# klausondrag/FOSVOS

Measured on AMD Instinct MI355X. Metric: online fine-tune frames/sec (854x480), higher is better.
Workload: dtype bf16; 1 GPU; OSVOS_VGG train_online one-shot fine-tune: 1x3x480x854 frame per step, fwd + class-balanced BCE + bwd, fused SGD step every 5 steps (BASELINE.json configs[1]); batch=1, avg_grad_every_n=5, activations=bf16 NHWC, fp32 accumulate, fp32 master weights, parallelism=single GPU

## Files before the change

### fosvos_amd/csrc/common.hpp

```cpp
#pragma once
#include <hip/hip_runtime.h>
#include <stdarg.h>
#include <algorithm>
#include <stdint.h>
#include <stdio.h>
#include <stdlib.h>
#include <string.h>

#include "../../include/fosvos_hip.h"

namespace fosvos {

extern thread_local char g_err[512];

inline int fail(int code, const char *fmt, ...) __attribute__((format(printf, 2, 3)));
inline int fail(int code, const char *fmt, ...) {
    va_list ap;
    va_start(ap, fmt);
    vsnprintf(g_err, sizeof(g_err), fmt, ap);
    va_end(ap);
    return code;
}

#define FOSVOS_HIP_CHECK(expr)                                                                         \
    do {                                                                                               \
        hipError_t e_ = (expr);                                                                        \
        if (e_ != hipSuccess)                                                                          \
            return ::fosvos::fail(FOSVOS_E_HIP, "%s: %s (%s:%d)", #expr, hipGetErrorString(e_), __FILE__, \
                                  __LINE__);                                                           \
    } while (0)

#define FOSVOS_REQUIRE(cond, code, ...)                    \
    do {                                                   \
        if (!(cond)) return ::fosvos::fail(code, __VA_ARGS__); \
    } while (0)

#define FOSVOS_ENTER(device) FOSVOS_HIP_CHECK(hipSetDevice(device))
extern bool g_prof_on;
void prof_begin(const char *name, hipStream_t st, double flops);
void prof_end();
#define FOSVOS_PROF(name, st, flops)                                        \
    do {                                                                    \
        if (::fosvos::g_prof_on) ::fosvos::prof_begin(name, (hipStream_t)(st), flops); \
    } while (0)
#define FOSVOS_LAUNCH_CHECK()                            \
    do {                                                 \
        if (::fosvos::g_prof_on) ::fosvos::prof_end();   \
        FOSVOS_HIP_CHECK(hipGetLastError());             \
    } while (0)

struct WgradReduceEntry {
    const float *slabs;
    float *dw, *db;
    const float *bias_part;
    int64_t E_real, E_pad;
    int S, S_bias, Co, Cor, accumulate;
    int block_begin, n_blocks;
    int fold_begin, fold_blocks;
};
constexpr int kWgradReduceMax = 20;
struct WgradReduceTable {
    int n;
    WgradReduceEntry e[kWgradReduceMax];
};
int wgrad_impl(const uint16_t *x, const uint16_t *dy, float *dw, float *db, int N, int H, int W, int Ci, int Co,
               int accumulate, void *workspace, size_t workspace_bytes, int device, void *stream,
               WgradReduceTable *reduce, bool alone = false);
int first_wgrad_impl(const float *frame, const uint16_t *dy, float *dw, float *db, int N, int H, int W, int Co,
                     int accumulate, void *workspace, size_t workspace_bytes, int device, void *stream,
                     WgradReduceTable *reduce);
int wgrad_reduce_all(WgradReduceTable *reduce, int device, void *stream);
int wgrad_queue_reduce(const float *slabs, const float *bias_part, float *dw, float *db, int S, int S_bias, int64_t E_real,
                       int64_t E_pad, int Co, int Cor, int accumulate, WgradReduceTable *reduce, int device, void *stream);
struct HeadBwdArgs {
    const float *const *side;
    const int *hs, *ws;
    const float *const *filt, *const *filt1;
    const float *dsn_w, *fuse_w, *d_fused;
    const float *const *d_side_out;
    uint16_t *const *d_side;
    float *d_fuse_w, *d_fuse_b, *d_dsn_w, *d_dsn_b;
    int N, H, W, accumulate;
    void *workspace;
    size_t workspace_bytes;
    int device;
    int filt_uniform;
};
int head_bwd_check(const HeadBwdArgs &a);
int head_bwd_scale(const HeadBwdArgs &a, int s, void *stream);
int head_bwd_finish(const HeadBwdArgs &a, void *stream);

}
constexpr int kFosvosVggEvents = 25, kFosvosResnetEvents = 12;
struct fosvos_ctx {
    uint32_t magic;
    int device;
    hipEvent_t vgg_ev[kFosvosVggEvents];
    hipEvent_t resnet_ev[kFosvosResnetEvents];
    bool buckets_recorded;
};
constexpr uint32_t kFosvosCtxMagic = 0x58544346u;
namespace fosvos {
inline int ctx_check(const fosvos_ctx *ctx, const char *who) {
    FOSVOS_REQUIRE(ctx != nullptr, FOSVOS_E_ARG, "%s: null context (fosvos_ctx_create)", who);
    FOSVOS_REQUIRE(ctx->magic == kFosvosCtxMagic, FOSVOS_E_ARG, "%s: not a live fosvos_ctx", who);
    return FOSVOS_OK;
}

#ifdef FOSVOS_LAB_BUILD
inline const char *lab_env(const char *name) { return getenv(name); }
#else
// ... 158 lines not shown
```

### fosvos_amd/csrc/conv_wgrad.hip

```cpp
#include <stdlib.h>

#include "common.hpp"

using namespace fosvos;

namespace {
constexpr int TH = 8;
constexpr int TPIX = TH * 16;
constexpr int HALO_W = 18;
constexpr int BCI = 64;

struct WgArgs {
    const uint16_t *x;
    const uint16_t *dy;
    float *slabs;
    float *bias_part;
    int N, H, W, Ci, Cy, Cor;
    int tiles_x, tiles_y, n_tiles, tiles_per_split;
    int lab;
    int S, n_ci, n_co, xcd_order;
};

typedef __attribute__((address_space(3))) s16x4 *lds_s16x4_ptr;

// ... 205 lines not shown
            if constexpr ((R) < 4) {                                                                                \
                _Pragma("unroll") for (int kx = 0; kx < 3; ++kx)                                                    \
                _Pragma("unroll") for (int u = 0; u < NU; ++u)                                                      \
                    acc[kx][u] = __builtin_amdgcn_mfma_f32_16x16x32_bf16(a0[u], b[kx], acc[kx][u], 0, 0, 0);        \
                if (my_bias) {                                                                                      \
                    _Pragma("unroll") for (int u = 0; u < NU; ++u) bsum[u] = add8(a0[u], bsum[u]);                  \
                }                                                                                                   \
            }                                                                                                       \
            asm volatile("" ::: "memory");                                                                          \
            b[0] = bn[0]; b[1] = bn[1]; b[2] = bn[2];                                                               \
        }
        FOSVOS_W2_ROW(0) FOSVOS_W2_ROW(1) FOSVOS_W2_ROW(2) FOSVOS_W2_ROW(3) FOSVOS_W2_ROW(4) FOSVOS_W2_ROW(5)
        if (has_next) FOSVOS_W2_ADVANCE()
        asm volatile("s_waitcnt vmcnt(0)" ::: "memory");
        __syncthreads();
    }

    if (do_bias) {
        float *sb = reinterpret_cast<float *>(smem_w);
#pragma unroll
        for (int u = 0; u < NU; ++u) sb[(wi * 4 + g) * C::BCO + wc * 32 + u * 16 + (lane & 15)] = bsum[u];
        __syncthreads();
        if (tid < C::BCO && co0 + tid < a.Cor) {
            float acc_b = 0.f;
#pragma unroll
            for (int k = 0; k < 16; ++k) acc_b += sb[k * C::BCO + tid];
            a.bias_part[((int64_t)split * a.n_ci + ci_blk) * a.Cor + co0 + tid] = acc_b;
        }
    }
    float *slab = a.slabs + (int64_t)split * a.Cor * a.Ci * 9;
    const int ci = ci0 + wi * 16 + (lane & 15);
#pragma unroll
    for (int u = 0; u < NU; ++u)
#pragma unroll
        for (int r = 0; r < 4; ++r) {
            const int co = co0 + wc * 32 + u * 16 + 4 * g + r;
            if (co >= a.Cor || (a.lab & 1)) continue;
            float *d = slab + ((int64_t)co * a.Ci + ci) * 9;
#pragma unroll
            for (int t = 0; t < 9; ++t) d[t] = acc[t][u][r];
        }
#undef FOSVOS_W2_ROW
#undef FOSVOS_W2_PIECES_OF_ROW
#undef FOSVOS_W2_PIECE_ANY
#undef FOSVOS_W2_TILE_SCALARS
#undef FOSVOS_W2_ADVANCE
#undef FOSVOS_W2_STAGE
#undef FOSVOS_W2_PIECE_X
#undef FOSVOS_W2_PIECE_Y
}
}

constexpr int kFold = 8;

__global__ __launch_bounds__(256) void k_wgrad_fold(const WgradReduceTable t) {
    int e = 0;
    while (e + 1 < t.n && (int)blockIdx.x >= t.e[e + 1].fold_begin) ++e;
    const WgradReduceEntry &q = t.e[e];
    const int local = blockIdx.x - q.fold_begin;
    if (local >= q.fold_blocks) return;
    const int per_group = q.n_blocks;
    const int grp = local / per_group;
    const int64_t i4 = (int64_t)(local - grp * per_group) * 256 + threadIdx.x;
    if (i4 * 4 >= q.E_real) return;
    float *base = const_cast<float *>(q.slabs) + (int64_t)grp * kFold * q.E_pad + i4 * 4;
    const int n = min(kFold, q.S - grp * kFold);
    float4 v[kFold];
#pragma unroll
    for (int j = 0; j < kFold; ++j) v[j] = *reinterpret_cast<const float4 *>(base + (int64_t)min(j, n - 1) * q.E_pad);
    float4 acc = v[0];
#pragma unroll
    for (int j = 1; j < kFold; ++j)
        if (j < n) { acc.x += v[j].x; acc.y += v[j].y; acc.z += v[j].z; acc.w += v[j].w; }
    *reinterpret_cast<float4 *>(base) = acc;
}

__global__ __launch_bounds__(256) void k_wgrad_reduce(const WgradReduceTable t) {
    int e = 0;
    while (e + 1 < t.n && (int)blockIdx.x >= t.e[e + 1].block_begin) ++e;
    const WgradReduceEntry &q = t.e[e];
    const int local = blockIdx.x - q.block_begin;
    const int64_t i4 = (int64_t)local * 256 + threadIdx.x;
    const bool folded = q.fold_blocks > 0;
    const int n_src = folded ? (q.S + kFold - 1) / kFold : q.S;
    const int64_t stride = (folded ? kFold : 1) * q.E_pad;
    if (i4 * 4 < q.E_real) {
        const float *src = q.slabs + i4 * 4;
        float4 acc = make_float4(0.f, 0.f, 0.f, 0.f);
        for (int s0 = 0; s0 < n_src; s0 += 8) {
            float4 v[8];
#pragma unroll
            for (int j = 0; j < 8; ++j) v[j] = *reinterpret_cast<const float4 *>(src + (int64_t)min(s0 + j, n_src - 1) * stride);
#pragma unroll
            for (int j = 0; j < 8; ++j)
                if (s0 + j < n_src) { acc.x += v[j].x; acc.y += v[j].y; acc.z += v[j].z; acc.w += v[j].w; }
        }
        float4 *d = reinterpret_cast<float4 *>(q.dw + i4 * 4);
        if (q.accumulate) {
            const float4 o = *d;
            acc.x += o.x; acc.y += o.y; acc.z += o.z; acc.w += o.w;
        }
        *d = acc;
    }
    if (local == 0 && q.db) {
        __shared__ float s_part[256];
        int Cg = 1;
        while (Cg < q.Co && Cg < 256) Cg <<= 1;
        const int P = 256 / Cg, part = threadIdx.x / Cg, cl = threadIdx.x - part * Cg;
        const int per = (q.S_bias + P - 1) / P, s_lo = part * per, s_hi = min(s_lo + per, q.S_bias);
        for (int co0 = 0; co0 < q.Co; co0 += Cg) {
            const int co = co0 + cl;
            float acc_b = 0.f;
            if (co < q.Co) {
                for (int s0 = s_lo; s0 < s_hi; s0 += 16) {
                    float v[16];
#pragma unroll
                    for (int j = 0; j < 16; ++j) v[j] = q.bias_part[(int64_t)min(s0 + j, s_hi - 1) * q.Cor + co];
#pragma unroll
                    for (int j = 0; j < 16; ++j)
                        if (s0 + j < s_hi) acc_b += v[j];
                }
            }
            if (co0) __syncthreads();
            s_part[threadIdx.x] = acc_b;
            __syncthreads();
            if (part == 0 && co < q.Co) {
                float t = s_part[cl];
                for (int pp = 1; pp < P; ++pp) t += s_part[pp * Cg + cl];
                q.db[co] = q.accumulate ? q.db[co] + t : t;
            }
        }
    }
}

int target_blocks() {
    static const int v = [] {
        const char *e = lab_env("FOSVOS_WGRAD_BLOCKS");
        const int n = e ? atoi(e) : 0;
        return n > 0 ? n : 192;
    }();
    return v;
}

struct Plan {
    int Cor, Cy, side, tiles_x, tiles_y, n_tiles, tps, S, n_ci;
    size_t slab_bytes, bias_bytes;
};

Plan make_plan(int N, int H, int W, int Ci, int Co, bool alone = false) {
    Plan p;
    p.side = Co % 64 != 0;
    p.Cor = p.side ? Co : roundup(Co, 64);
    p.Cy = roundup(Co, 32);
    p.tiles_x = (int)cdiv(W, 16);
    p.tiles_y = (int)cdiv(H, TH);
    p.n_tiles = p.tiles_x * p.tiles_y * N;
    const int out_blocks = p.side ? Ci / 64 : (p.Cor / 64) * (Ci / 64);
    int S = (int)cdiv(alone ? std::max(256, target_blocks()) : target_blocks(), out_blocks);
    if (S > p.n_tiles) S = p.n_tiles;
    if (S < 1) S = 1;
    p.tps = (int)cdiv(p.n_tiles, S);
    p.S = (int)cdiv(p.n_tiles, p.tps);
    p.slab_bytes = (size_t)p.S * 9 * p.Cor * Ci * sizeof(float);
    p.n_ci = Ci / 64;
    p.bias_bytes = (size_t)p.S * p.n_ci * p.Cor * sizeof(float);
    return p;
}

int check_shape(int N, int H, int W, int Ci, int Co, const char *who) {
    FOSVOS_REQUIRE(N > 0 && H > 0 && W > 0 && Ci > 0 && Co > 0, FOSVOS_E_SHAPE, "%s: bad shape", who);
    FOSVOS_REQUIRE(Ci % BCI == 0, FOSVOS_E_SHAPE, "%s: Ci=%d must be a multiple of %d", who, Ci, BCI);
    FOSVOS_REQUIRE(Co % 64 == 0 || Co == 16, FOSVOS_E_SHAPE, "%s: Co=%d must be a multiple of 64, or 16 (side_prep)", who, Co);
    FOSVOS_REQUIRE(((int64_t)N * H * W + W + 1) * std::max(Ci, roundup(Co, 32)) * 2 < 0xffffffffLL, FOSVOS_E_SHAPE,
                   "%s: a tensor of %d x %d x %d x %d bf16 exceeds the 4 GB a buffer descriptor addresses", who, N, H, W,
                   std::max(Ci, roundup(Co, 32)));
    return FOSVOS_OK;
}

int finish_or_queue(const Plan &p, float *slabs, float *bias_part, float *dw, float *db, int Ci, int Co, int accumulate,
                    WgradReduceTable *reduce, int device, hipStream_t st) {
    return fosvos::wgrad_queue_reduce(slabs, bias_part, dw, db, p.S, p.S * p.n_ci, 9LL * Co * Ci, 9LL * p.Cor * Ci, Co, p.Cor,
                                      accumulate, reduce, device, st);
}
}

extern "C" size_t fosvos_conv3x3_wgrad_workspace_bytes(int N, int H, int W, int Ci, int Co) {
    if (N <= 0 || H <= 0 || W <= 0 || Ci <= 0 || Co <= 0 || Ci % BCI != 0) return 0;
    const Plan p = make_plan(N, H, W, Ci, Co), q = make_plan(N, H, W, Ci, Co, true);
    return std::max(p.slab_bytes + p.bias_bytes, q.slab_bytes + q.bias_bytes);
}

extern "C" int fosvos_conv3x3_wgrad(const uint16_t *x, const uint16_t *dy, float *dw, float *db, int N, int H, int W,
                                    int Ci, int Co, int accumulate, void *workspace, size_t workspace_bytes, int device,
                                    void *stream) {
    return fosvos::wgrad_impl(x, dy, dw, db, N, H, W, Ci, Co, accumulate, workspace, workspace_bytes, device, stream,
                              nullptr);
}

extern "C" int fosvos_conv3x3_wgrad_reduce(float *dw, float *db, int N, int H, int W, int Ci, int Co, int accumulate,
                                           void *workspace, size_t workspace_bytes, int device, void *stream) {
    FOSVOS_REQUIRE(dw && workspace, FOSVOS_E_ARG, "conv3x3_wgrad_reduce: null pointer");
    if (int rc = check_shape(N, H, W, Ci, Co, "conv3x3_wgrad_reduce")) return rc;
    const Plan p = make_plan(N, H, W, Ci, Co);
    FOSVOS_REQUIRE(workspace_bytes >= p.slab_bytes + p.bias_bytes, FOSVOS_E_WORKSPACE,
                   "conv3x3_wgrad_reduce: workspace %zu < %zu", workspace_bytes, p.slab_bytes + p.bias_bytes);
    FOSVOS_ENTER(device);
    float *slabs = reinterpret_cast<float *>(workspace);
    float *bias_part = reinterpret_cast<float *>(reinterpret_cast<char *>(workspace) + p.slab_bytes);
    return finish_or_queue(p, slabs, bias_part, dw, db, Ci, Co, accumulate, nullptr, device, (hipStream_t)stream);
}

extern "C" int fosvos_conv3x3_wgrad_slabs(const uint16_t *x, const uint16_t *dy, int with_bias, int N, int H, int W, int Ci,
                                          int Co, void *workspace, size_t workspace_bytes, int device, void *stream) {
    WgradReduceTable sink;
    sink.n = 0;
    float dummy = 0.f;
    return fosvos::wgrad_impl(x, dy, &dummy, with_bias ? &dummy : nullptr, N, H, W, Ci, Co, 0, workspace, workspace_bytes,
                              device, stream, &sink);
}

int fosvos::wgrad_queue_reduce(const float *slabs, const float *bias_part, float *dw, float *db, int S, int S_bias,
                               int64_t E_real,
                               int64_t E_pad, int Co, int Cor, int accumulate, WgradReduceTable *reduce, int device,
                               void *stream) {
    WgradReduceTable local;
    local.n = 0;
    WgradReduceTable *t = reduce ? reduce : &local;
    FOSVOS_REQUIRE(t->n < kWgradReduceMax, FOSVOS_E_ARG, "wgrad: reduction queue full");
    FOSVOS_REQUIRE(E_real % 4 == 0 && E_pad % 4 == 0, FOSVOS_E_SHAPE, "wgrad: slab size must be a multiple of 4 floats");
    WgradReduceEntry &q = t->e[t->n];
    q.slabs = slabs; q.dw = dw; q.db = db; q.bias_part = db ? bias_part : nullptr;
    q.S = S; q.S_bias = S_bias; q.Co = Co; q.Cor = Cor; q.accumulate = accumulate;
    q.E_real = E_real;
    q.E_pad = E_pad;
    q.n_blocks = (int)cdiv(E_real / 4, 256);
    q.block_begin = t->n ? t->e[t->n - 1].block_begin + t->e[t->n - 1].n_blocks : 0;
    q.fold_blocks = S > kFold ? (int)cdiv(S, kFold) * q.n_blocks : 0;
    q.fold_begin = t->n ? t->e[t->n - 1].fold_begin + t->e[t->n - 1].fold_blocks : 0;
    ++t->n;
    return reduce ? FOSVOS_OK : fosvos::wgrad_reduce_all(t, device, stream);
}

int fosvos::wgrad_reduce_all(WgradReduceTable *reduce, int device, void *stream) {
    FOSVOS_REQUIRE(reduce, FOSVOS_E_ARG, "wgrad_reduce_all: null table");
    if (reduce->n == 0) return FOSVOS_OK;
    FOSVOS_ENTER(device);
    const WgradReduceEntry &last = reduce->e[reduce->n - 1];
    if (last.fold_begin + last.fold_blocks > 0) {
        FOSVOS_PROF("k_wgrad_fold", stream, 0.0);
        hipLaunchKernelGGL(k_wgrad_fold, dim3((unsigned)(last.fold_begin + last.fold_blocks)), dim3(256), 0,
                           (hipStream_t)stream, *reduce);
        FOSVOS_LAUNCH_CHECK();
    }
    FOSVOS_PROF("k_wgrad_reduce", stream, 0.0);
    hipLaunchKernelGGL(k_wgrad_reduce, dim3((unsigned)(last.block_begin + last.n_blocks)), dim3(256), 0, (hipStream_t)stream,
                       *reduce);
    FOSVOS_LAUNCH_CHECK();
    reduce->n = 0;
    return FOSVOS_OK;
}

int fosvos::wgrad_impl(const uint16_t *x, const uint16_t *dy, float *dw, float *db, int N, int H, int W, int Ci, int Co,
                       int accumulate, void *workspace, size_t workspace_bytes, int device, void *stream,
                       WgradReduceTable *reduce, bool alone) {
    FOSVOS_REQUIRE(x && dy && dw && workspace, FOSVOS_E_ARG, "conv3x3_wgrad: null pointer");
    if (int rc = check_shape(N, H, W, Ci, Co, "conv3x3_wgrad")) return rc;
    const Plan p = make_plan(N, H, W, Ci, Co, alone);
    FOSVOS_REQUIRE(workspace_bytes >= p.slab_bytes + p.bias_bytes, FOSVOS_E_WORKSPACE,
                   "conv3x3_wgrad: workspace %zu < %zu", workspace_bytes, p.slab_bytes + p.bias_bytes);
    FOSVOS_ENTER(device);
    hipStream_t st = (hipStream_t)stream;
    WgArgs a;
    a.x = x; a.dy = dy; a.slabs = reinterpret_cast<float *>(workspace);
    a.bias_part = db ? reinterpret_cast<float *>(reinterpret_cast<char *>(workspace) + p.slab_bytes) : nullptr;
    a.N = N; a.H = H; a.W = W; a.Ci = Ci; a.Cy = p.Cy; a.Cor = p.Cor;
    a.tiles_x = p.tiles_x; a.tiles_y = p.tiles_y; a.n_tiles = p.n_tiles; a.tiles_per_split = p.tps;
    a.S = p.S; a.n_ci = Ci / 64; a.n_co = p.side ? 1 : p.Cor / 64;
    {
#ifdef FOSVOS_LAB_BUILD
        static const int lab = lab_env_int("FOSVOS_WGRAD_LAB", 0);
        a.lab = lab;
#else
        a.lab = 0;
#endif
        const char *e = lab_env("FOSVOS_WGRAD_XCD");
        a.xcd_order = !(e && atoi(e) == 0);
    }
    static bool once[64][2];
    const double flops = 2.0 * N * H * W * 9.0 * Ci * Co;
    const dim3 grid((unsigned)(p.S * a.n_ci * a.n_co));
    if (p.side) {
        using C2 = v2::Cfg2<true>;
        if (device >= 0 && device < 64 && !once[device][1]) {
            FOSVOS_HIP_CHECK(hipFuncSetAttribute(reinterpret_cast<const void *>(v2::k_wgrad3x3_v2<true>),
                                                 hipFuncAttributeMaxDynamicSharedMemorySize, C2::LDS_BYTES));
            once[device][1] = true;
        }
        FOSVOS_PROF("k_wgrad3x3_v2<true>", st, flops);
        hipLaunchKernelGGL(v2::k_wgrad3x3_v2<true>, grid, dim3(C2::NT), C2::LDS_BYTES, st, a);
    } else {
        using C2 = v2::Cfg2<false>;
        if (device >= 0 && device < 64 && !once[device][0]) {
            FOSVOS_HIP_CHECK(hipFuncSetAttribute(reinterpret_cast<const void *>(v2::k_wgrad3x3_v2<false>),
                                                 hipFuncAttributeMaxDynamicSharedMemorySize, C2::LDS_BYTES));
            once[device][0] = true;
        }
        FOSVOS_PROF("k_wgrad3x3_v2<false>", st, flops);
        hipLaunchKernelGGL(v2::k_wgrad3x3_v2<false>, grid, dim3(C2::NT), C2::LDS_BYTES, st, a);
    }
// ... 4 lines not shown
```

### fosvos_amd/fosvos_hip/__init__.py

```python
from __future__ import annotations

import ctypes
import os
import threading
from ctypes import POINTER, c_char_p, c_float, c_int, c_int64, c_size_t, c_uint, c_void_p

_HERE = os.path.dirname(os.path.abspath(__file__))
PKG_ROOT = os.path.dirname(_HERE)
LIB_PATH = os.environ.get("FOSVOS_HIP_LIB") or os.path.join(PKG_ROOT, "lib", "libfosvos_hip.so")
HEADER_PATH = os.path.join(os.path.dirname(PKG_ROOT), "include", "fosvos_hip.h")

ABI_VERSION = 33
CONV_RELU = 1
CONV_OUT_F32 = 2
VGG_COMPACT_STAGE1 = 1


class FosvosHipError(RuntimeError):
    pass


class SgdEntry(ctypes.Structure):
    _fields_ = [("param", c_void_p), ("grad", c_void_p), ("momentum_buf", c_void_p), ("numel", c_int64),
                ("lr", c_float), ("weight_decay", c_float)]
# ... 54 lines not shown
                ("kind", c_int)]


class ResnetBlock(ctypes.Structure):
    _fields_ = [("conv", Conv2dDesc * 3), ("n_convs", c_int), ("has_down", c_int), ("down", Conv2dDesc)]


class ResnetNet(ctypes.Structure):
    _fields_ = [("first_w", c_void_p), ("first_b", c_void_p), ("first_co", c_int), ("first_fp32_math", c_int), ("first_unfused", c_int),
                ("blocks_per_stage", c_int * 4),
                ("blocks", POINTER(ResnetBlock)), ("side", Conv2dDesc * 4), ("filt", c_void_p * 4),
                ("filt1", c_void_p * 4), ("stride", c_int * 4), ("dsn_w", c_void_p), ("dsn_b", c_void_p),
                ("fuse_b", c_void_p)]

SIGNATURES = {
    "fosvos_abi_version": (c_int, []),
    "fosvos_last_error": (c_char_p, []),
    "fosvos_build_arch": (c_char_p, []),
    "fosvos_ctx_create": (c_int, [c_int, POINTER(c_void_p)]),
    "fosvos_ctx_destroy": (c_int, [c_void_p]),
    "fosvos_ctx_device": (c_int, [c_void_p]),
    "fosvos_conv3x3_plan": (c_int, [c_int, c_int, c_int, c_int, c_int, POINTER(Conv3x3PlanInfo)]),
    "fosvos_conv3x3_fwd_plan": (c_int, [c_int, c_int, c_int, c_int, c_int, ctypes.c_uint, POINTER(Conv3x3PlanInfo)]),
    "fosvos_conv3x3_first_plan": (c_int, [c_int, c_int, c_int, POINTER(c_int), POINTER(c_int)]),
    "fosvos_nchw_f32_to_nhwc_bf16": (c_int, [c_void_p, c_void_p, c_int, c_int, c_int, c_int, c_int, c_int, c_void_p]),
    "fosvos_nhwc_bf16_to_nchw_f32": (c_int, [c_void_p, c_void_p, c_int, c_int, c_int, c_int, c_int, c_int, c_void_p]),
    "fosvos_nhwc_f32_to_nchw_f32": (c_int, [c_void_p, c_void_p, c_int, c_int, c_int, c_int, c_int, c_void_p]),
    "fosvos_nchw_f32_to_nhwc_f32": (c_int, [c_void_p, c_void_p, c_int, c_int, c_int, c_int, c_int, c_void_p]),
    "fosvos_pack_conv3x3_weights": (c_int, [c_void_p, c_int, c_int, c_void_p, c_void_p, c_int, c_void_p]),
    "fosvos_packed_weight_elems": (c_size_t, [c_int, c_int]),
    "fosvos_pack_conv3x3_weights_multi": (c_int, [POINTER(PackEntry), c_int, c_int, c_void_p]),
    "fosvos_conv3x3_first_fwd": (c_int, [c_void_p, c_void_p, c_void_p, c_void_p, c_void_p, c_int, c_int, c_int, c_int, c_int,
                                         c_void_p]),
    "fosvos_conv3x3_dgrad_bits": (c_int, [c_void_p, c_void_p, c_void_p, c_void_p, c_void_p, c_int, c_int, c_int, c_int,
                                          c_int, c_void_p, c_size_t, c_int, c_void_p]),
    "fosvos_conv3x3_dgrad_unpool": (c_int, [c_void_p, c_void_p, c_void_p, c_void_p, c_void_p, c_int, c_int, c_int, c_int,
                                            c_int, c_void_p, c_size_t, c_int, c_void_p]),
    "fosvos_conv3x3_first_wgrad": (c_int, [c_void_p, c_void_p, c_void_p, c_void_p, c_int, c_int, c_int, c_int,
                                           c_void_p, c_size_t, c_int, c_void_p]),
    "fosvos_conv3x3_first_wgrad_workspace_bytes": (c_size_t, [c_int, c_int, c_int, c_int]),
    "fosvos_conv3x3_fwd": (c_int, [c_void_p, c_void_p, c_void_p, c_void_p, c_int, c_int, c_int, c_int, c_int, c_uint,
                                   c_void_p, c_size_t, c_int, c_void_p]),
    "fosvos_conv3x3_fwd_pool": (c_int, [c_void_p, c_void_p, c_void_p, c_void_p, c_void_p, c_int, c_int, c_int, c_int,
                                        c_int, c_uint, c_void_p, c_size_t, c_int, c_void_p]),
    "fosvos_conv3x3_workspace_bytes": (c_size_t, [c_int, c_int, c_int, c_int, c_int]),
    "fosvos_conv3x3_dgrad": (c_int, [c_void_p, c_void_p, c_void_p, c_void_p, c_void_p, c_int, c_int, c_int, c_int,
                                     c_int, c_void_p, c_size_t, c_int, c_void_p]),
    "fosvos_conv3x3_wgrad": (c_int, [c_void_p, c_void_p, c_void_p, c_void_p, c_int, c_int, c_int, c_int, c_int, c_int,
                                     c_void_p, c_size_t, c_int, c_void_p]),
    "fosvos_conv3x3_wgrad_slabs": (c_int, [c_void_p, c_void_p, c_int, c_int, c_int, c_int, c_int, c_int, c_void_p, c_size_t,
                                           c_int, c_void_p]),
    "fosvos_conv3x3_wgrad_reduce": (c_int, [c_void_p, c_void_p, c_int, c_int, c_int, c_int, c_int, c_int, c_void_p,
                                            c_size_t, c_int, c_void_p]),
    "fosvos_conv3x3_wgrad_workspace_bytes": (c_size_t, [c_int, c_int, c_int, c_int, c_int]),
    "fosvos_maxpool2x2_ceil_fwd": (c_int, [c_void_p, c_void_p, c_int, c_int, c_int, c_int, c_int, c_void_p]),
    "fosvos_maxpool2x2_ceil_bwd": (c_int, [c_void_p, c_void_p, c_void_p, c_int, c_int, c_int, c_int, c_int, c_int,
                                           c_void_p]),
    "fosvos_head_fwd": (c_int, [POINTER(c_void_p), POINTER(c_int), POINTER(c_int), POINTER(c_void_p),
                                POINTER(c_void_p), c_void_p, c_void_p, c_void_p, c_void_p, c_void_p,
                                POINTER(c_void_p), c_int, c_int, c_int, c_int, c_int, c_void_p]),
    "fosvos_head_bwd": (c_int, [POINTER(c_void_p), POINTER(c_int), POINTER(c_int), POINTER(c_void_p),
                                POINTER(c_void_p), c_void_p, c_void_p, c_void_p, POINTER(c_void_p),
                                POINTER(c_void_p), c_void_p, c_void_p, c_void_p, c_void_p, c_int, c_int, c_int, c_int,
                                c_void_p, c_size_t, c_int, c_void_p]),
    "fosvos_head_bwd_workspace_bytes": (c_size_t, [c_int, c_int, c_int]),
    "fosvos_cbce_loss": (c_int, [c_void_p, c_void_p, c_int64, c_int, c_float, c_void_p, c_void_p, c_void_p, c_size_t,
                                 c_int, c_void_p]),
    "fosvos_cbce_workspace_bytes": (c_size_t, [c_int64]),
    "fosvos_cbce_loss_frames": (c_int, [c_void_p, c_void_p, c_int64, c_int, c_int, c_float, c_void_p, c_void_p, c_void_p,
                                        c_size_t, c_int, c_void_p]),
    "fosvos_cbce_loss_frames_parts": (c_int, [c_void_p, c_void_p, c_int64, c_int, c_int, c_float, c_void_p, c_void_p,
                                              c_void_p, c_size_t, c_int, c_int, c_void_p]),
    "fosvos_cbce_multi_workspace_bytes": (c_size_t, [c_int64, c_int, c_int]),
    "fosvos_cbce_loss_frames_multi": (c_int, [POINTER(c_void_p), c_void_p, c_int64, c_int, c_int, c_int, POINTER(c_float),
                                              c_void_p, POINTER(c_void_p), c_void_p, c_size_t, c_int, c_int, c_void_p]),
    "fosvos_cbce_loss_batch_counts": (c_int, [c_void_p, c_void_p, c_int64, c_int, c_float, c_void_p, c_void_p, c_void_p,
                                              c_void_p, c_size_t, c_int, c_void_p]),
    "fosvos_sgd_momentum_step": (c_int, [c_void_p, c_int, c_int64, c_float, c_int, c_int, c_void_p]),
    "fosvos_conv3x3_s2_fwd": (c_int, [c_void_p, c_void_p, c_void_p, c_void_p, c_int, c_int, c_int, c_int, c_int, c_uint,
                                      c_void_p, c_size_t, c_int, c_void_p]),
    "fosvos_conv3x3_fwd_add": (c_int, [c_void_p, c_void_p, c_void_p, c_void_p, c_void_p, c_int, c_int, c_int, c_int, c_int,
                                       c_uint, c_void_p, c_size_t, c_int, c_void_p]),
    "fosvos_fold_conv_bn": (c_int, [c_void_p, c_int, c_int, c_int, c_void_p, c_void_p, c_void_p, c_void_p, c_void_p,
                                    c_float, c_void_p, c_void_p, c_int, c_void_p]),
    "fosvos_conv2d_packed_dwords": (c_size_t, [c_int, c_int, c_int]),
    "fosvos_conv2d_bias_elems": (c_size_t, [c_int]),
    "fosvos_pack_conv2d_bn": (c_int, [c_void_p, c_int, c_int, c_int, c_void_p, c_void_p, c_void_p, c_void_p, c_void_p,
                                      c_float, c_void_p, c_void_p, c_int, c_void_p]),
    "fosvos_conv2d_plan": (c_int, [c_int, c_int, c_int, c_int, c_int, c_int, c_int, POINTER(Conv2dPlanInfo)]),
    "fosvos_conv2d_fwd": (c_int, [c_void_p, c_void_p, c_void_p, c_void_p, c_void_p, c_int, c_int, c_int, c_int, c_int,
                                  c_int, c_int, c_uint, c_int, c_void_p]),
    "fosvos_conv7x7_packed_elems": (c_size_t, [c_int]),
    "fosvos_pack_conv7x7_bn": (c_int, [c_void_p, c_int, c_void_p, c_void_p, c_void_p, c_void_p, c_float, c_void_p,
                                       c_void_p, c_int, c_void_p]),
    "fosvos_conv7x7s2_first_fwd": (c_int, [c_void_p, c_void_p, c_void_p, c_void_p, c_int, c_int, c_int, c_int, c_uint,
                                           c_int, c_void_p]),
    "fosvos_conv7x7s2_pool_first_fwd": (c_int, [c_void_p, c_void_p, c_void_p, c_void_p, c_int, c_int, c_int, c_int, c_int,
                                                c_void_p]),
    "fosvos_maxpool3x3s2_fwd": (c_int, [c_void_p, c_void_p, c_int, c_int, c_int, c_int, c_int, c_void_p]),
    "fosvos_deconv_head_fwd": (c_int, [POINTER(c_void_p), POINTER(c_int), POINTER(c_int), POINTER(c_int),
                                       POINTER(c_void_p), POINTER(c_void_p), c_void_p, c_void_p, c_void_p, c_void_p,
                                       POINTER(c_void_p), c_int, c_int, c_int, c_int, c_void_p]),
    "fosvos_resnet_arena_bytes": (c_size_t, [POINTER(ResnetNet), c_int, c_int, c_int]),
    "fosvos_resnet_forward": (c_int, [POINTER(ResnetNet), c_void_p, c_int, c_int, c_int, c_void_p, c_size_t, c_void_p,
                                      POINTER(c_void_p), c_int, c_void_p, c_void_p, c_void_p]),
    "fosvos_vgg_arena_bytes": (c_size_t, [c_int, c_int, c_int]),
# ... 162 lines not shown
```

### fosvos_amd/fosvos_hip/ops.py

```python
from __future__ import annotations

from typing import List, Optional, Sequence, Tuple

import torch

from . import CONV_OUT_F32, CONV_RELU, check, int_array4, lib, ptr_array4

_BF16 = torch.bfloat16
_F32 = torch.float32


def _need(t: torch.Tensor, dtype, what: str) -> torch.Tensor:
    if not t.is_cuda:
        raise RuntimeError(f"{what}: tensor must live on the GPU (the HIP path has no CPU fallback)")
    if t.dtype != dtype:
        raise TypeError(f"{what}: expected {dtype}, got {t.dtype}")
    if not t.is_contiguous():
        raise ValueError(f"{what}: tensor must be contiguous")
    return t


def _ctx(t: torch.Tensor) -> Tuple[int, int]:
    dev = t.device.index if t.device.index is not None else torch.cuda.current_device()
    return dev, torch.cuda.current_stream(dev).cuda_stream
# ... 351 lines not shown
        _need(out, _BF16, "conv3x3_dgrad_unpool out")
        if tuple(out.shape) != (n, h, wd, ci) or out.data_ptr() == x.data_ptr():
            raise ValueError("conv3x3_dgrad_unpool: out must have x's shape and must not alias it")
    dx = out if out is not None else torch.empty((n, h, wd, ci), dtype=_BF16, device=dy.device)
    ws, wsn = _WS.get(L.fosvos_conv3x3_workspace_bytes(n, h, wd, co, ci), dy.device)
    dev, st = _ctx(dy)
    t0 = _pb()
    check(L.fosvos_conv3x3_dgrad_unpool(dy.data_ptr(), w_dgrad_packed.data_ptr(), x.data_ptr(), d_pooled.data_ptr(), dx.data_ptr(),
                                        n, h, wd, ci, co, ws, wsn, dev, st), "conv3x3_dgrad_unpool")
    _pe(t0, "conv3x3_dgrad_unpool", 2.0 * n * h * wd * 9 * ci * co, n * h * wd * 2 * (cy + 2 * ci + ci // 4) + 2 * 9 * ci * co)
    return dx


def conv3x3_wgrad(x: torch.Tensor, dy: torch.Tensor, ci: int, co: int, with_bias: bool = True,
                  dw: Optional[torch.Tensor] = None, db: Optional[torch.Tensor] = None, accumulate: bool = False):
    _need(x, _BF16, "conv3x3_wgrad x"); _need(dy, _BF16, "conv3x3_wgrad dy")
    n, h, wd, cx = x.shape
    if cx != ci or tuple(dy.shape) != (n, h, wd, _ru(co, 32)):
        raise ValueError(f"conv3x3_wgrad: shapes x={tuple(x.shape)} dy={tuple(dy.shape)} do not match Ci={ci} Co={co}")
    L = lib()
    if dw is None:
        if accumulate:
            raise ValueError("conv3x3_wgrad: accumulate needs an existing dw")
        dw = torch.empty((co, ci, 3, 3), dtype=_F32, device=x.device)
    if with_bias and db is None:
        if accumulate:
            raise ValueError("conv3x3_wgrad: accumulate needs an existing db")
        db = torch.empty((co,), dtype=_F32, device=x.device)
    _need(dw, _F32, "conv3x3_wgrad dw")
    ws, wsn = _WS.get(L.fosvos_conv3x3_wgrad_workspace_bytes(n, h, wd, ci, co), x.device)
    dev, st = _ctx(x)
    t0 = _pb()
    check(L.fosvos_conv3x3_wgrad_slabs(x.data_ptr(), dy.data_ptr(), 1 if with_bias else 0, n, h, wd, ci, co, ws, wsn, dev, st),
          "conv3x3_wgrad_slabs")
    _pe(t0, "conv3x3_wgrad", 2.0 * n * h * wd * 9 * ci * co, n * h * wd * 2 * (ci + dy.shape[3]))
    t0 = _pb()
    check(L.fosvos_conv3x3_wgrad_reduce(dw.data_ptr(), _p(db) if with_bias else None, n, h, wd, ci, co,
                                        1 if accumulate else 0, ws, wsn, dev, st), "conv3x3_wgrad_reduce")
    _pe(t0, "wgrad_reduce", 0.0, 4 * 9 * ci * co * 3)
    return dw, (db if with_bias else None)


def conv3x3_wgrad_one_call(x: torch.Tensor, dy: torch.Tensor, ci: int, co: int, with_bias: bool = True):
    _need(x, _BF16, "conv3x3_wgrad x"); _need(dy, _BF16, "conv3x3_wgrad dy")
    n, h, wd, _ = x.shape
    L = lib()
    dw = torch.empty((co, ci, 3, 3), dtype=_F32, device=x.device)
    db = torch.empty((co,), dtype=_F32, device=x.device) if with_bias else None
    ws, wsn = _WS.get(L.fosvos_conv3x3_wgrad_workspace_bytes(n, h, wd, ci, co), x.device)
    dev, st = _ctx(x)
    check(L.fosvos_conv3x3_wgrad(x.data_ptr(), dy.data_ptr(), dw.data_ptr(), _p(db), n, h, wd, ci, co, 0, ws, wsn, dev, st),
          "conv3x3_wgrad")
    return dw, db


def maxpool_fwd(x: torch.Tensor) -> torch.Tensor:
    _need(x, _BF16, "maxpool_fwd")
    n, h, w, c = x.shape
    y = torch.empty((n, (h + 1) // 2, (w + 1) // 2, c), dtype=_BF16, device=x.device)
    dev, st = _ctx(x)
    t0 = _pb()
    check(lib().fosvos_maxpool2x2_ceil_fwd(x.data_ptr(), y.data_ptr(), n, h, w, c, dev, st), "maxpool2x2_ceil_fwd")
    _pe(t0, "maxpool_fwd", 0.0, 2 * (x.numel() + y.numel()))
    return y


def maxpool_bwd(x: torch.Tensor, dy: torch.Tensor, relu_mask: bool = True) -> torch.Tensor:
    _need(x, _BF16, "maxpool_bwd x"); _need(dy, _BF16, "maxpool_bwd dy")
    n, h, w, c = x.shape
    if tuple(dy.shape) != (n, (h + 1) // 2, (w + 1) // 2, c):
        raise ValueError("maxpool_bwd: dy shape mismatch")
    dx = torch.empty_like(x)
    dev, st = _ctx(x)
    t0 = _pb()
    check(lib().fosvos_maxpool2x2_ceil_bwd(x.data_ptr(), dy.data_ptr(), dx.data_ptr(), n, h, w, c, 1 if relu_mask else 0,
                                           dev, st), "maxpool2x2_ceil_bwd")
    _pe(t0, "maxpool_bwd", 0.0, 2 * (2 * x.numel() + dy.numel()))
    return dx


def maxpool_bwd_codes(codes: torch.Tensor, dy: torch.Tensor, h: int, w: int, out: Optional[torch.Tensor] = None) -> torch.Tensor:
    _need(dy, _BF16, "maxpool_bwd_codes dy")
    n, oh, ow, c = dy.shape
    if (oh, ow) != ((h + 1) // 2, (w + 1) // 2) or c % 8:
        raise ValueError("maxpool_bwd_codes: dy shape mismatch")
    if not (codes.is_cuda and codes.is_contiguous() and codes.dtype == torch.int32) or codes.numel() != n * oh * ow * (c // 8):
        raise ValueError("maxpool_bwd_codes: codes must be a contiguous int32 [N, ceil(h/2), ceil(w/2), C/8] tensor on the GPU")
    dx = torch.empty((n, h, w, c), dtype=_BF16, device=dy.device) if out is None else out
    if out is not None:
        _need(out, _BF16, "maxpool_bwd_codes out")
        if out.numel() != n * h * w * c:
            raise ValueError("maxpool_bwd_codes: out size")
    dev, st = _ctx(dy)
    t0 = _pb()
    check(lib().fosvos_maxpool2x2_ceil_bwd_codes(codes.data_ptr(), dy.data_ptr(), dx.data_ptr(), n, h, w, c, dev, st),
          "maxpool2x2_ceil_bwd_codes")
    _pe(t0, "maxpool_bwd", 0.0, 2 * (dx.numel() + dy.numel()) + 4 * codes.numel())
    return dx


def vgg_stage1_compact(n: int, h: int, w: int, flag: bool = True) -> bool:
    from . import VGG_COMPACT_STAGE1
    return bool(lib().fosvos_vgg_stage1_compact(VGG_COMPACT_STAGE1 if flag else 0, n, h, w))


def head_fwd(side: Sequence[torch.Tensor], filt: Sequence[torch.Tensor], filt1: Optional[Sequence[torch.Tensor]],
# ... 1412 lines not shown
```

### include/fosvos_hip.h

```cpp
#ifndef FOSVOS_HIP_H
#define FOSVOS_HIP_H

#include <stddef.h>
#include <stdint.h>

#ifdef __cplusplus
extern "C" {
#endif

#define FOSVOS_ABI_VERSION 33

#define FOSVOS_OK 0
#define FOSVOS_E_SHAPE (-1)
#define FOSVOS_E_ARG (-2)
#define FOSVOS_E_WORKSPACE (-3)
#define FOSVOS_E_HIP (-4)

#define FOSVOS_CONV_RELU 1u
#define FOSVOS_CONV_OUT_F32 2u
#define FOSVOS_CONV_FP32_MATH 4u

int fosvos_abi_version(void);

typedef struct fosvos_profile_record {
// ... 41 lines not shown
    int Co, Ci;
} fosvos_pack_entry;
int fosvos_pack_conv3x3_weights_multi(const fosvos_pack_entry *entries, int n, int device, void *stream);

int fosvos_conv3x3_first_fwd(const float *frame, const float *w_oihw, const float *bias, uint16_t *y, uint8_t *relu_bits,
                             int N, int H, int W, int Co, int device, void *stream);
int fosvos_conv3x3_first_plan(int N, int H, int W, int *tiles, int *workgroups);
int fosvos_conv3x3_first_wgrad(const float *frame, const uint16_t *dy, float *dw_oihw, float *dbias, int N, int H,
                               int W, int Co, void *workspace, size_t workspace_bytes, int device, void *stream);
size_t fosvos_conv3x3_first_wgrad_workspace_bytes(int N, int H, int W, int Co);

int fosvos_conv3x3_fwd(const uint16_t *x, const uint16_t *w_packed, const float *bias, void *y, int N, int H, int W,
                       int Ci, int Co, unsigned flags, void *workspace, size_t workspace_bytes, int device,
                       void *stream);

int fosvos_conv3x3_s2_fwd(const uint16_t *x, const uint16_t *w_packed, const float *bias, uint16_t *y, int N, int H, int W,
                          int Ci, int Co, unsigned flags, void *workspace, size_t workspace_bytes, int device, void *stream);
int fosvos_conv3x3_fwd_add(const uint16_t *x, const uint16_t *w_packed, const float *bias, const uint16_t *addend,
                           void *y, int N, int H, int W, int Ci, int Co, unsigned flags, void *workspace,
                           size_t workspace_bytes, int device, void *stream);
int fosvos_conv3x3_fwd_pool(const uint16_t *x, const uint16_t *w_packed, const float *bias, uint16_t *y,
                            uint16_t *y_pool, int N, int H, int W, int Ci, int Co, unsigned flags, void *workspace,
                            size_t workspace_bytes, int device, void *stream);
int fosvos_conv3x3_fwd_pool_codes(const uint16_t *x, const uint16_t *w_packed, const float *bias, uint16_t *y_pool,
                                  uint32_t *codes, int N, int H, int W, int Ci, int Co, unsigned flags, int device,
                                  void *stream);
size_t fosvos_conv3x3_pool_codes_bytes(int N, int H, int W, int C);
size_t fosvos_conv3x3_workspace_bytes(int N, int H, int W, int in_ch, int out_ch);
typedef struct fosvos_conv3x3_plan_info {
    int tile_h, tile_w, tile_co;
    int k_splits;
    int workgroups;
    int persistent;
} fosvos_conv3x3_plan_info;
int fosvos_conv3x3_plan(int N, int H, int W, int in_ch, int out_ch, fosvos_conv3x3_plan_info *out);
int fosvos_conv3x3_fwd_plan(int N, int H, int W, int in_ch, int out_ch, unsigned flags, fosvos_conv3x3_plan_info *out);
int fosvos_conv3x3_dgrad(const uint16_t *dy, const uint16_t *w_dgrad_packed, const uint16_t *relu_src,
                         const uint16_t *addend, uint16_t *dx, int N, int H, int W, int Ci, int Co, void *workspace,
                         size_t workspace_bytes, int device, void *stream);
int fosvos_conv3x3_dgrad_bits(const uint16_t *dy, const uint16_t *w_dgrad_packed, const uint8_t *relu_bits,
                              const uint16_t *addend, uint16_t *dx, int N, int H, int W, int Ci, int Co, void *workspace,
                              size_t workspace_bytes, int device, void *stream);
int fosvos_conv3x3_dgrad_unpool(const uint16_t *dy, const uint16_t *w_dgrad_packed, const uint16_t *x,
                                const uint16_t *d_pooled, uint16_t *dx, int N, int H, int W, int Ci, int Co,
                                void *workspace, size_t workspace_bytes, int device, void *stream);
int fosvos_conv3x3_wgrad(const uint16_t *x, const uint16_t *dy, float *dw_oihw, float *dbias, int N, int H, int W,
                         int Ci, int Co, int accumulate, void *workspace, size_t workspace_bytes, int device,
                         void *stream);
size_t fosvos_conv3x3_wgrad_workspace_bytes(int N, int H, int W, int Ci, int Co);
int fosvos_conv3x3_wgrad_slabs(const uint16_t *x, const uint16_t *dy, int with_bias, int N, int H, int W, int Ci, int Co,
                               void *workspace, size_t workspace_bytes, int device, void *stream);
int fosvos_conv3x3_wgrad_reduce(float *dw_oihw, float *dbias, int N, int H, int W, int Ci, int Co, int accumulate,
                                void *workspace, size_t workspace_bytes, int device, void *stream);

int fosvos_maxpool2x2_ceil_fwd(const uint16_t *x, uint16_t *y, int N, int H, int W, int C, int device, void *stream);
int fosvos_maxpool2x2_ceil_bwd(const uint16_t *x, const uint16_t *dy, uint16_t *dx, int N, int H, int W, int C,
                               int relu_mask, int device, void *stream);
int fosvos_maxpool2x2_ceil_bwd_codes(const uint32_t *codes, const uint16_t *dy, uint16_t *dx, int N, int H, int W, int C,
                                     int device, void *stream);

int fosvos_head_fwd(const float *const side[4], const int hs[4], const int ws[4], const float *const filt[4],
                    const float *const filt1[4], const float *dsn_w , const float *dsn_b ,
                    const float *fuse_w , const float *fuse_b , float *fused,
                    float *const side_out[4] , int N, int H, int W, int filt_uniform, int device,
                    void *stream);
int fosvos_head_bwd(const float *const side[4], const int hs[4], const int ws[4], const float *const filt[4],
                    const float *const filt1[4], const float *dsn_w, const float *fuse_w, const float *d_fused,
                    const float *const d_side_out[4], uint16_t *const d_side[4], float *d_fuse_w, float *d_fuse_b,
                    float *d_dsn_w, float *d_dsn_b, int N, int H, int W, int filt_uniform ,
                    void *workspace, size_t workspace_bytes, int device, void *stream);
size_t fosvos_head_bwd_workspace_bytes(int N, int H, int W);

int fosvos_cbce_loss(const float *logits, const float *label, int64_t numel, int size_average, float grad_scale,
                     float *loss_out, float *grad, void *workspace, size_t workspace_bytes, int device,
                     void *stream);
size_t fosvos_cbce_workspace_bytes(int64_t numel);
int fosvos_cbce_loss_frames(const float *logits, const float *label, int64_t frame_numel, int n_frames, int size_average,
                            float grad_scale, float *loss_out, float *grad, void *workspace, size_t workspace_bytes,
                            int device, void *stream);
#define FOSVOS_CBCE_COUNT 1
#define FOSVOS_CBCE_LOSS 2
#define FOSVOS_CBCE_FINISH 4
int fosvos_cbce_loss_frames_parts(const float *logits, const float *label, int64_t frame_numel, int n_frames,
                                  int size_average, float grad_scale, float *loss_out, float *grad, void *workspace,
                                  size_t workspace_bytes, int parts, int device, void *stream);
#define FOSVOS_CBCE_MAX_MAPS 8
size_t fosvos_cbce_multi_workspace_bytes(int64_t frame_numel, int n_frames, int n_maps);
int fosvos_cbce_loss_frames_multi(const float *const *logits, const float *label, int64_t frame_numel, int n_frames,
                                  int n_maps, int size_average, const float *map_scale, float *loss_out, float *const *grad,
                                  void *workspace, size_t workspace_bytes, int parts, int device, void *stream);
int fosvos_cbce_loss_batch_counts(const float *logits, const float *label, int64_t numel, int size_average,
                                  float grad_scale, const double *batch_counts, float *loss_out, float *grad,
                                  void *workspace, size_t workspace_bytes, int device, void *stream);
size_t fosvos_cbce_void_workspace_bytes(int64_t frame_numel, int n_frames);
int fosvos_cbce_loss_frames_void(const float *logits, const float *label, const uint8_t *void_px, int64_t frame_numel,
                                 int n_frames, int size_average, float grad_scale, float *loss_out, float *grad,
                                 void *workspace, size_t workspace_bytes, int device, void *stream);

#define FOSVOS_SGD_FIRST_STEP 1
#define FOSVOS_SGD_ZERO_GRAD 2
typedef struct fosvos_sgd_entry {
    float *param;
    const float *grad;
    float *momentum_buf;
    int64_t numel;
    float lr;
// ... 206 lines not shown
```

Measured before the change: 1283 frames/s.

## Fuse wgrad slab fold and reduce into one multi-lane kernel

```diff
diff --git a/fosvos_amd/csrc/common.hpp b/fosvos_amd/csrc/common.hpp
--- a/fosvos_amd/csrc/common.hpp
+++ b/fosvos_amd/csrc/common.hpp
@@ -56,7 +56,7 @@
     int64_t E_real, E_pad;
     int S, S_bias, Co, Cor, accumulate;
     int block_begin, n_blocks;
-    int fold_begin, fold_blocks;
+    int lanes;
 };
 constexpr int kWgradReduceMax = 20;
 struct WgradReduceTable {
diff --git a/fosvos_amd/csrc/conv_wgrad.hip b/fosvos_amd/csrc/conv_wgrad.hip
--- a/fosvos_amd/csrc/conv_wgrad.hip
+++ b/fosvos_amd/csrc/conv_wgrad.hip
@@ -281,85 +281,99 @@
 }
 
 constexpr int kFold = 8;
-
-__global__ __launch_bounds__(256) void k_wgrad_fold(const WgradReduceTable t) {
-    int e = 0;
-    while (e + 1 < t.n && (int)blockIdx.x >= t.e[e + 1].fold_begin) ++e;
-    const WgradReduceEntry &q = t.e[e];
-    const int local = blockIdx.x - q.fold_begin;
-    if (local >= q.fold_blocks) return;
-    const int per_group = q.n_blocks;
-    const int grp = local / per_group;
-    const int64_t i4 = (int64_t)(local - grp * per_group) * 256 + threadIdx.x;
-    if (i4 * 4 >= q.E_real) return;
-    float *base = const_cast<float *>(q.slabs) + (int64_t)grp * kFold * q.E_pad + i4 * 4;
-    const int n = min(kFold, q.S - grp * kFold);
-    float4 v[kFold];
-#pragma unroll
-    for (int j = 0; j < kFold; ++j) v[j] = *reinterpret_cast<const float4 *>(base + (int64_t)min(j, n - 1) * q.E_pad);
-    float4 acc = v[0];
-#pragma unroll
-    for (int j = 1; j < kFold; ++j)
-        if (j < n) { acc.x += v[j].x; acc.y += v[j].y; acc.z += v[j].z; acc.w += v[j].w; }
-    *reinterpret_cast<float4 *>(base) = acc;
-}
-
-__global__ __launch_bounds__(256) void k_wgrad_reduce(const WgradReduceTable t) {
+constexpr int kReduceThreads = 1024, kReduceMaxLanes = 32;
+
+__device__ __forceinline__ void add4(float4 &a, const float4 &b) { a.x += b.x; a.y += b.y; a.z += b.z; a.w += b.w; }
+
+__device__ __forceinline__ void reduce_bias(const WgradReduceEntry &q, float *s_part) {
+    const bool act = threadIdx.x < 256;
+    int Cg = 1;
+    while (Cg < q.Co && Cg < 256) Cg <<= 1;
+    const int P = 256 / Cg, part = threadIdx.x / Cg, cl = threadIdx.x - part * Cg;
+    const int per = (q.S_bias + P - 1) / P, s_lo = part * per, s_hi = min(s_lo + per, q.S_bias);
+    for (int co0 = 0; co0 < q.Co; co0 += Cg) {
+        const int co = co0 + cl;
+        float acc_b = 0.f;
+        if (act && co < q.Co) {
+            for (int s0 = s_lo; s0 < s_hi; s0 += 16) {
+                float v[16];
+#pragma unroll
+                for (int j = 0; j < 16; ++j) v[j] = q.bias_part[(int64_t)min(s0 + j, s_hi - 1) * q.Cor + co];
+#pragma unroll
+                for (int j = 0; j < 16; ++j)
+                    if (s0 + j < s_hi) acc_b += v[j];
+            }
+        }
+        if (co0) __syncthreads();
+        if (act) s_part[threadIdx.x] = acc_b;
+        __syncthreads();
+        if (act && part == 0 && co < q.Co) {
+            float t = s_part[cl];
+            for (int pp = 1; pp < P; ++pp) t += s_part[pp * Cg + cl];
+            q.db[co] = q.accumulate ? q.db[co] + t : t;
+        }
+    }
+}
+
+__global__ __launch_bounds__(kReduceThreads) void k_wgrad_reduce(const WgradReduceTable t) {
+    __shared__ float4 s_g[kReduceThreads];
     int e = 0;
     while (e + 1 < t.n && (int)blockIdx.x >= t.e[e + 1].block_begin) ++e;
     const WgradReduceEntry &q = t.e[e];
-    const int local = blockIdx.x - q.block_begin;
-    const int64_t i4 = (int64_t)local * 256 + threadIdx.x;
-    const bool folded = q.fold_blocks > 0;
-    const int n_src = folded ? (q.S + kFold - 1) / kFold : q.S;
-    const int64_t stride = (folded ? kFold : 1) * q.E_pad;
-    if (i4 * 4 < q.E_real) {
-        const float *src = q.slabs + i4 * 4;
-        float4 acc = make_float4(0.f, 0.f, 0.f, 0.f);
-        for (int s0 = 0; s0 < n_src; s0 += 8) {
-            float4 v[8];
-#pragma unroll
-            for (int j = 0; j < 8; ++j) v[j] = *reinterpret_cast<const float4 *>(src + (int64_t)min(s0 + j, n_src - 1) * stride);
-#pragma unroll
-            for (int j = 0; j < 8; ++j)
-                if (s0 + j < n_src) { acc.x += v[j].x; acc.y += v[j].y; acc.z += v[j].z; acc.w += v[j].w; }
-        }
-        float4 *d = reinterpret_cast<float4 *>(q.dw + i4 * 4);
-        if (q.accumulate) {
-            const float4 o = *d;
-            acc.x += o.x; acc.y += o.y; acc.z += o.z; acc.w += o.w;
-        }
-        *d = acc;
-    }
-    if (local == 0 && q.db) {
-        __shared__ float s_part[256];
-        int Cg = 1;
-        while (Cg < q.Co && Cg < 256) Cg <<= 1;
-        const int P = 256 / Cg, part = threadIdx.x / Cg, cl = threadIdx.x - part * Cg;
-        const int per = (q.S_bias + P - 1) / P, s_lo = part * per, s_hi = min(s_lo + per, q.S_bias);
-        for (int co0 = 0; co0 < q.Co; co0 += Cg) {
-            const int co = co0 + cl;
-            float acc_b = 0.f;
-            if (co < q.Co) {
-                for (int s0 = s_lo; s0 < s_hi; s0 += 16) {
-                    float v[16];
-#pragma unroll
-                    for (int j = 0; j < 16; ++j) v[j] = q.bias_part[(int64_t)min(s0 + j, s_hi - 1) * q.Cor + co];
-#pragma unroll
-                    for (int j = 0; j < 16; ++j)
-                        if (s0 + j < s_hi) acc_b += v[j];
-                }
+    int local = blockIdx.x - q.block_begin;
+    if (q.db) {
+        if (local == 0) {
+            reduce_bias(q, reinterpret_cast<float *>(s_g));
+            return;
+        }
+        --local;
+    }
+    const int L = q.lanes, F = kReduceThreads / L;
+    const int lane = threadIdx.x / F, el = threadIdx.x - lane * F;
+    const int64_t i4 = (int64_t)local * F + el;
+    const bool valid = i4 * 4 < q.E_real;
+    const bool owner = valid && lane == 0;
+    const float *src = q.slabs + i4 * 4;
+    float4 *d = reinterpret_cast<float4 *>(q.dw + i4 * 4);
+    float4 old = make_float4(0.f, 0.f, 0.f, 0.f);
+    if (owner && q.accumulate) old = *d;
+    float4 acc = make_float4(0.f, 0.f, 0.f, 0.f);
+    if (L == 1) {
+        if (valid) {
+            float4 v[kFold];
+#pragma unroll
+            for (int j = 0; j < kFold; ++j) v[j] = *reinterpret_cast<const float4 *>(src + (int64_t)min(j, q.S - 1) * q.E_pad);
+#pragma unroll
+            for (int j = 0; j < kFold; ++j)
+                if (j < q.S) add4(acc, v[j]);
+        }
+    } else {
+        const int G = (q.S + kFold - 1) / kFold;
+        for (int g0 = 0; g0 < G; g0 += L) {
+            const int grp = g0 + lane;
+            if (valid && grp < G) {
+                const float *base = src + (int64_t)grp * kFold * q.E_pad;
+                const int n = min(kFold, q.S - grp * kFold);
+                float4 v[kFold];
+#pragma unroll
+                for (int j = 0; j < kFold; ++j) v[j] = *reinterpret_cast<const float4 *>(base + (int64_t)min(j, n - 1) * q.E_pad);
+                float4 g = v[0];
+#pragma unroll
+                for (int j = 1; j < kFold; ++j)
+                    if (j < n) add4(g, v[j]);
+                s_g[threadIdx.x] = g;
             }
-            if (co0) __syncthreads();
-            s_part[threadIdx.x] = acc_b;
             __syncthreads();
-            if (part == 0 && co < q.Co) {
-                float t = s_part[cl];
-                for (int pp = 1; pp < P; ++pp) t += s_part[pp * Cg + cl];
-                q.db[co] = q.accumulate ? q.db[co] + t : t;
+            if (owner) {
+                const int m = min(L, G - g0);
+                for (int k = 0; k < m; ++k) add4(acc, s_g[k * F + el]);
             }
-        }
-    }
+            if (g0 + L < G) __syncthreads();
+        }
+    }
+    if (!owner) return;
+    if (q.accumulate) add4(acc, old);
+    *d = acc;
 }
 
 int target_blocks() {
@@ -448,6 +462,19 @@
                               device, stream, &sink);
 }
 
+extern "C" int fosvos_wgrad_reduce_slabs(const float *slabs, const float *bias_part, float *dw, float *db, int S, int S_bias,
+                                         int64_t E_real, int64_t E_pad, int Co, int Cor, int accumulate, int device,
+                                         void *stream) {
+    FOSVOS_REQUIRE(slabs && dw && (!db || bias_part), FOSVOS_E_ARG, "wgrad_reduce_slabs: null pointer");
+    FOSVOS_REQUIRE(S >= 1 && (!db || S_bias >= 1), FOSVOS_E_SHAPE, "wgrad_reduce_slabs: S=%d S_bias=%d", S, S_bias);
+    FOSVOS_REQUIRE(E_real > 0 && E_real <= E_pad && E_real % 4 == 0 && E_pad % 4 == 0, FOSVOS_E_SHAPE,
+                   "wgrad_reduce_slabs: E_real=%lld E_pad=%lld must be multiples of 4 with E_real <= E_pad",
+                   (long long)E_real, (long long)E_pad);
+    FOSVOS_REQUIRE(Co >= 1 && Co <= Cor, FOSVOS_E_SHAPE, "wgrad_reduce_slabs: Co=%d Cor=%d", Co, Cor);
+    return fosvos::wgrad_queue_reduce(slabs, bias_part, dw, db, S, S_bias, E_real, E_pad, Co, Cor, accumulate, nullptr, device,
+                                      stream);
+}
+
 int fosvos::wgrad_queue_reduce(const float *slabs, const float *bias_part, float *dw, float *db, int S, int S_bias,
                                int64_t E_real,
                                int64_t E_pad, int Co, int Cor, int accumulate, WgradReduceTable *reduce, int device,
@@ -462,10 +489,11 @@
     q.S = S; q.S_bias = S_bias; q.Co = Co; q.Cor = Cor; q.accumulate = accumulate;
     q.E_real = E_real;
     q.E_pad = E_pad;
-    q.n_blocks = (int)cdiv(E_real / 4, 256);
+    q.lanes = 1;
+    if (S > kFold)
+        while (q.lanes < kReduceMaxLanes && q.lanes * kFold < S) q.lanes <<= 1;
+    q.n_blocks = (db ? 1 : 0) + (int)cdiv(E_real / 4, kReduceThreads / q.lanes);
     q.block_begin = t->n ? t->e[t->n - 1].block_begin + t->e[t->n - 1].n_blocks : 0;
-    q.fold_blocks = S > kFold ? (int)cdiv(S, kFold) * q.n_blocks : 0;
-    q.fold_begin = t->n ? t->e[t->n - 1].fold_begin + t->e[t->n - 1].fold_blocks : 0;
     ++t->n;
     return reduce ? FOSVOS_OK : fosvos::wgrad_reduce_all(t, device, stream);
 }
@@ -475,15 +503,9 @@
     if (reduce->n == 0) return FOSVOS_OK;
     FOSVOS_ENTER(device);
     const WgradReduceEntry &last = reduce->e[reduce->n - 1];
-    if (last.fold_begin + last.fold_blocks > 0) {
-        FOSVOS_PROF("k_wgrad_fold", stream, 0.0);
-        hipLaunchKernelGGL(k_wgrad_fold, dim3((unsigned)(last.fold_begin + last.fold_blocks)), dim3(256), 0,
-                           (hipStream_t)stream, *reduce);
-        FOSVOS_LAUNCH_CHECK();
-    }
     FOSVOS_PROF("k_wgrad_reduce", stream, 0.0);
-    hipLaunchKernelGGL(k_wgrad_reduce, dim3((unsigned)(last.block_begin + last.n_blocks)), dim3(256), 0, (hipStream_t)stream,
-                       *reduce);
+    hipLaunchKernelGGL(k_wgrad_reduce, dim3((unsigned)(last.block_begin + last.n_blocks)), dim3(kReduceThreads), 0,
+                       (hipStream_t)stream, *reduce);
     FOSVOS_LAUNCH_CHECK();
     reduce->n = 0;
     return FOSVOS_OK;
diff --git a/fosvos_amd/fosvos_hip/__init__.py b/fosvos_amd/fosvos_hip/__init__.py
--- a/fosvos_amd/fosvos_hip/__init__.py
+++ b/fosvos_amd/fosvos_hip/__init__.py
@@ -130,6 +130,8 @@
                                            c_int, c_void_p]),
     "fosvos_conv3x3_wgrad_reduce": (c_int, [c_void_p, c_void_p, c_int, c_int, c_int, c_int, c_int, c_int, c_void_p,
                                             c_size_t, c_int, c_void_p]),
+    "fosvos_wgrad_reduce_slabs": (c_int, [c_void_p, c_void_p, c_void_p, c_void_p, c_int, c_int, c_int64, c_int64, c_int, c_int,
+                                          c_int, c_int, c_void_p]),
     "fosvos_conv3x3_wgrad_workspace_bytes": (c_size_t, [c_int, c_int, c_int, c_int, c_int]),
     "fosvos_maxpool2x2_ceil_fwd": (c_int, [c_void_p, c_void_p, c_int, c_int, c_int, c_int, c_int, c_void_p]),
     "fosvos_maxpool2x2_ceil_bwd": (c_int, [c_void_p, c_void_p, c_void_p, c_int, c_int, c_int, c_int, c_int, c_int,
diff --git a/fosvos_amd/fosvos_hip/ops.py b/fosvos_amd/fosvos_hip/ops.py
--- a/fosvos_amd/fosvos_hip/ops.py
+++ b/fosvos_amd/fosvos_hip/ops.py
@@ -427,6 +427,25 @@
     check(L.fosvos_conv3x3_wgrad(x.data_ptr(), dy.data_ptr(), dw.data_ptr(), _p(db), n, h, wd, ci, co, 0, ws, wsn, dev, st),
           "conv3x3_wgrad")
     return dw, db
+
+
+def wgrad_reduce_slabs(slabs: torch.Tensor, dw: torch.Tensor, e_real: int, bias_part: Optional[torch.Tensor] = None,
+                       db: Optional[torch.Tensor] = None, co: int = 1, accumulate: bool = False) -> None:
+    _need(slabs, _F32, "wgrad_reduce_slabs slabs"); _need(dw, _F32, "wgrad_reduce_slabs dw")
+    if slabs.dim() != 2 or dw.numel() < e_real:
+        raise ValueError("wgrad_reduce_slabs: slabs must be [S, E_pad] and dw hold e_real elements")
+    s_bias, cor = 0, co
+    if db is not None:
+        if bias_part is None:
+            raise ValueError("wgrad_reduce_slabs: db needs bias_part")
+        _need(bias_part, _F32, "wgrad_reduce_slabs bias_part"); _need(db, _F32, "wgrad_reduce_slabs db")
+        if bias_part.dim() != 2 or db.numel() < co:
+            raise ValueError("wgrad_reduce_slabs: bias_part must be [S_bias, Cor] and db hold co elements")
+        s_bias, cor = bias_part.shape
+    dev, st = _ctx(slabs)
+    check(lib().fosvos_wgrad_reduce_slabs(slabs.data_ptr(), _p(bias_part) if db is not None else None, dw.data_ptr(), _p(db),
+                                          slabs.shape[0], s_bias, e_real, slabs.shape[1], co, cor, 1 if accumulate else 0,
+                                          dev, st), "wgrad_reduce_slabs")
 
 
 def maxpool_fwd(x: torch.Tensor) -> torch.Tensor:
diff --git a/include/fosvos_hip.h b/include/fosvos_hip.h
--- a/include/fosvos_hip.h
+++ b/include/fosvos_hip.h
@@ -117,6 +117,8 @@
                                void *workspace, size_t workspace_bytes, int device, void *stream);
 int fosvos_conv3x3_wgrad_reduce(float *dw_oihw, float *dbias, int N, int H, int W, int Ci, int Co, int accumulate,
                                 void *workspace, size_t workspace_bytes, int device, void *stream);
+int fosvos_wgrad_reduce_slabs(const float *slabs, const float *bias_part, float *dw, float *db, int S, int S_bias,
+                              int64_t E_real, int64_t E_pad, int Co, int Cor, int accumulate, int device, void *stream);
 
 int fosvos_maxpool2x2_ceil_fwd(const uint16_t *x, uint16_t *y, int N, int H, int W, int C, int device, void *stream);
 int fosvos_maxpool2x2_ceil_bwd(const uint16_t *x, const uint16_t *dy, uint16_t *dx, int N, int H, int W, int C,
```

After: 1283 frames/s. No clear change (-0.0%).
